# briangodwinlim/SIR-GCN

Measured on AMD Instinct MI355X. Metric: edges/sec SIRConv fwd+bwd, d_hidden=256, 1/2/4/8 MI355X, higher is better.
Workload: dtype f32; 1 GPU; cfg4 S2: Chung-Lu power-law V=2000000 E=40000000 alpha=0.8; 1 SIRConv layer d_in=H=d_out=256, agg=sum, LeakyReLU(0.2), f32, feat_dropout=0.0; fwd+bwd incl. projections; graph=S2, V=2000000, E=40000000, hidden=256, agg=sum, parallelism=single GPU

## Files before the change

### sir-gcn_amd/csrc/sirconv_gemm.hip

```cpp
#include <type_traits>
#include <algorithm>

#include "sirconv_internal.h"
#include "sirconv_gemm_util.h"
#include "sirconv_dropout.h"

namespace sir {
namespace {
using namespace gemm;

typedef _Float16 h8 __attribute__((ext_vector_type(8)));
typedef float f16v __attribute__((ext_vector_type(16)));
typedef unsigned int u4v __attribute__((ext_vector_type(4)));

constexpr int KC = 32;

#ifndef SIR_HR
#define SIR_HR 8
#endif

__device__ inline int bexp(float m) { return (int)((__float_as_uint(m) >> 23) & 255u) - 126; }
__device__ inline int scale_exp(int e) { int s = 15 - e; return s > 126 ? 126 : s; }
constexpr int SE_INIT = 127;
__device__ inline int next_se(int se_old, int e_c) {
    if (e_c + se_old <= 15) return se_old;
    const int s = 15 - SIR_HR - e_c;
    return s > 126 ? 126 : s;
}
__device__ inline void kahan_add(float& s, float& c, float x) {
    const float y = x - c;
    const float t = s + y;
    c = (t - s) - y;
    s = t;
}
__device__ inline float pow2(int e) { e = e < -126 ? -126 : (e > 127 ? 127 : e); return __uint_as_float((uint32_t)(e + 127) << 23); }
__device__ inline void drop4(const Drop& d, int64_t row, int n, float4& o) {
    const uint32_t rh = drop_row_hash(d, row);
    const int c = d.col0 + n;
    o.x = drop_keep(d, rh, c + 0) ? o.x * d.scale : 0.f;
    o.y = drop_keep(d, rh, c + 1) ? o.y * d.scale : 0.f;
    o.z = drop_keep(d, rh, c + 2) ? o.z * d.scale : 0.f;
    o.w = drop_keep(d, rh, c + 3) ? o.w * d.scale : 0.f;
}

__device__ inline float gate_dact(float g, float x, int relu, float slope) {
    return g > 0.f ? x : (relu ? 0.f : x * slope);
}
__global__ void __launch_bounds__(256)
k_gate_dact_bits(float* __restrict__ C, int64_t ldc, const uint64_t* __restrict__ mask, int64_t M, int relu, float slope) {
    const int64_t i = (int64_t)blockIdx.x * 256 + threadIdx.x;
    if (i >= M * 256) return;
    const int64_t r = i >> 8;
    const int c = (int)(i & 255);
    const bool pos = (mask[r * 4 + (c & 3)] >> (c >> 2)) & 1u;
    C[r * ldc + c] = gate_dact(pos ? 1.f : -1.f, C[r * ldc + c], relu, slope);
}
__global__ void __launch_bounds__(256)
k_gate_dact(float* __restrict__ C, int64_t ldc, const float* __restrict__ gate, int64_t M, int N, int relu, float slope) {
    const int64_t i = (int64_t)blockIdx.x * 256 + threadIdx.x;
    if (i >= M * N) return;
    const int64_t r = i / N, c = i % N;
    C[r * ldc + c] = gate_dact(gate[r * ldc + c], C[r * ldc + c], relu, slope);
}

__device__ inline void split8_mix(float4 a, float4 b, float s, h8& hi, h8& lo) {
    uint32_t h0, h1, h2, h3, l0, l1, l2, l3;
    asm volatile(
        "v_fma_mixlo_f16 %0, %8, %16, 0\n\tv_fma_mixhi_f16 %0, %9, %16, 0\n\t"
        "v_fma_mixlo_f16 %1, %10, %16, 0\n\tv_fma_mixhi_f16 %1, %11, %16, 0\n\t"
        "v_fma_mixlo_f16 %2, %12, %16, 0\n\tv_fma_mixhi_f16 %2, %13, %16, 0\n\t"
        "v_fma_mixlo_f16 %3, %14, %16, 0\n\tv_fma_mixhi_f16 %3, %15, %16, 0\n\t"
        "v_fma_mixlo_f16 %4, %8, %16, -%0 op_sel_hi:[0,0,1]\n\tv_fma_mixhi_f16 %4, %9, %16, -%0 op_sel:[0,0,1] op_sel_hi:[0,0,1]\n\t"
        "v_fma_mixlo_f16 %5, %10, %16, -%1 op_sel_hi:[0,0,1]\n\tv_fma_mixhi_f16 %5, %11, %16, -%1 op_sel:[0,0,1] op_sel_hi:[0,0,1]\n\t"
        "v_fma_mixlo_f16 %6, %12, %16, -%2 op_sel_hi:[0,0,1]\n\tv_fma_mixhi_f16 %6, %13, %16, -%2 op_sel:[0,0,1] op_sel_hi:[0,0,1]\n\t"
        "v_fma_mixlo_f16 %7, %14, %16, -%3 op_sel_hi:[0,0,1]\n\tv_fma_mixhi_f16 %7, %15, %16, -%3 op_sel:[0,0,1] op_sel_hi:[0,0,1]\n\t"
        "s_nop 1"
        : "=&v"(h0), "=&v"(h1), "=&v"(h2), "=&v"(h3), "=&v"(l0), "=&v"(l1), "=&v"(l2), "=&v"(l3)
        : "v"(a.x), "v"(a.y), "v"(a.z), "v"(a.w), "v"(b.x), "v"(b.y), "v"(b.z), "v"(b.w), "v"(s));
    typedef uint32_t u4 __attribute__((ext_vector_type(4)));
    hi = __builtin_bit_cast(h8, u4{h0, h1, h2, h3});
    lo = __builtin_bit_cast(h8, u4{l0, l1, l2, l3});
}
#define SIR_SPLIT1(x, i) { const float y_ = (x) * s; const _Float16 h_ = (_Float16)y_; hi[i] = h_; lo[i] = (_Float16)(y_ - (float)h_); }
__device__ inline void split8(float4 a, float4 b, float s, h8& hi, h8& lo) {
    SIR_SPLIT1(a.x, 0) SIR_SPLIT1(a.y, 1) SIR_SPLIT1(a.z, 2) SIR_SPLIT1(a.w, 3)
    SIR_SPLIT1(b.x, 4) SIR_SPLIT1(b.y, 5) SIR_SPLIT1(b.z, 6) SIR_SPLIT1(b.w, 7)
}
#undef SIR_SPLIT1

__device__ inline float fmax4_mix(float m, float4 v) {
    asm("v_max3_f32 %0, %0, |%1|, |%2|\n\tv_max3_f32 %0, %0, |%3|, |%4|" : "+v"(m) : "v"(v.x), "v"(v.y), "v"(v.z), "v"(v.w));
    return m;
}
__device__ inline float fmax4(float m, float4 v) {
    return fmaxf(fmaxf(m, fmaxf(fabsf(v.x), fabsf(v.y))), fmaxf(fabsf(v.z), fabsf(v.w)));
}

__global__ void __launch_bounds__(64)
k_pack_weight(const float* __restrict__ W, int64_t ldw, int N, int K, int trans, int Npad, int Kc,
              _Float16* __restrict__ out, float* __restrict__ inv_scale) {
    const int n = blockIdx.x, l = threadIdx.x;
    float m = 0.f;
    if (n < N)
        for (int k = l; k < K; k += 64) m = fmaxf(m, fabsf(trans ? W[(int64_t)k * ldw + n] : W[(int64_t)n * ldw + k]));
#pragma unroll
    for (int o = 32; o > 0; o >>= 1) m = fmaxf(m, __shfl_xor(m, o));
    const int se = scale_exp(bexp(m));
    const float s = pow2(se);
    for (int k = l; k < Kc * KC; k += 64) {
        float x = 0.f;
        if (n < N && k < K) x = trans ? W[(int64_t)k * ldw + n] : W[(int64_t)n * ldw + k];
        const float y = x * s;
        const _Float16 h = (_Float16)y;
        const int kc = k / KC, ks = (k / 16) & 1, j = k & 15;
        const int64_t at = fimg(n, j >> 3) / 2 + (j & 7);
        out[(((int64_t)kc * 2 + 0) * 2 + ks) * Npad * 16 + at] = h;
        out[(((int64_t)kc * 2 + 1) * 2 + ks) * Npad * 16 + at] = (_Float16)(y - (float)h);
    }
    if (l == 0) inv_scale[n] = (n < N) ? pow2(-se) : 0.f;
}

template <int WD, int WF, int TDT, int TFT, bool KFULL>
__global__ void __launch_bounds__(64 * WD * WF)
k_gemm_nt(const float* __restrict__ A, int64_t lda, int64_t M, int K,
          const u4v* __restrict__ Wp, int Npad, const float* __restrict__ inv_t,
          const float* __restrict__ bias, int N, float* __restrict__ C, int64_t ldc, int n_ftiles, Drop drop) {
    drop = drop_resolve(drop);
    constexpr int NT = 64 * WD * WF;
    constexpr int BD = 32 * TDT * WD;
    constexpr int BF = 32 * TFT * WF;
    constexpr int TPR = NT / BD;
    static_assert(TPR == 1 || TPR == 2 || TPR == 4, "loader mapping");
    constexpr int FPT = KC / TPR;
    constexpr int WPT = BF * 8 / NT;
    static_assert(WPT >= 1 && BF * 8 % NT == 0, "weight loader mapping");
    constexpr int D_BYTES = BD * 128, W_BYTES = BF * 128;
    constexpr int STAGE = D_BYTES + W_BYTES + BD * 4;
    __shared__ __attribute__((aligned(16))) char lds[2 * STAGE];

    const int t = threadIdx.x;
    const int wg = xcd_remap(blockIdx.x, gridDim.x);
    const int64_t d0 = (int64_t)(wg / n_ftiles) * BD;
    const int f0 = (wg % n_ftiles) * BF;
    const int nc = (K + KC - 1) / KC;

    const int rho = t / TPR, kp = t % TPR;
    const int64_t rows_here = (M - d0 < BD) ? M - d0 : BD;
    const rsrc_t arsrc = mk_rsrc(A + d0 * lda, (uint32_t)(rows_here * lda * 4));
    const int aoff = (rho * (int)lda + kp * FPT) * 4;
    const rsrc_t wrsrc = mk_rsrc(Wp, (uint32_t)((int64_t)nc * Npad * 128));
    int woff[WPT];
#pragma unroll
    for (int i = 0; i < WPT; ++i) {
        const int p = t + i * NT;
        const int plane = p / (BF * 2), rem = p % (BF * 2);
        const int nl = (rem >> 6) * 32 + (rem & 31), q = (rem >> 5) & 1;
        woff[i] = plane * Npad * 32 + fimg(f0 + nl, q);
    }
    int se_run = SE_INIT;

    const int w = t >> 6, l = t & 63, r = l & 31, h = l >> 5;
    const int d_w = (w / WF) * TDT * 32, f_w = (w % WF) * TFT * 32;

    float4 dv[2][FPT / 4];
    u4v wv[WPT];

    auto load_a = [&](int set, int c) {
#pragma unroll
        for (int i = 0; i < FPT / 4; ++i) {
            const int k = c * KC + kp * FPT + 4 * i;
            const u4v u = __builtin_amdgcn_raw_buffer_load_b128(arsrc, aoff + 16 * i, c * KC * 4, 0);
            dv[set][i] = (KFULL || k < K) ? make_float4(__uint_as_float(u.x), __uint_as_float(u.y), __uint_as_float(u.z),
                                               __uint_as_float(u.w))
                                 : make_float4(0.f, 0.f, 0.f, 0.f);
        }
    };
// ... 89 lines not shown
    store(0, 0, true);
    auto step_full = [&](int c, int set) {
        compute(c & 1);
        store(set, (c & 1) ^ 1);
        load_w(c + 2);
        load_a(set, c + 3);
        __syncthreads();
    };
    auto step_tail = [&](int c, int set) {
        compute(c & 1);
        if (c + 1 < nc) {
            store(set, (c & 1) ^ 1);
            if (c + 2 < nc) load_w(c + 2);
            if (c + 3 < nc) load_a(set, c + 3);
        }
        __syncthreads();
    };
    int c = 0;
    if (nc > 4) {
        load_a(1, 1);
        load_w(1);
        load_a(0, 2);
        __syncthreads();
        for (; c + 4 < nc; c += 2) {
            step_full(c, 1);
            step_full(c + 1, 0);
        }
    } else {
        if (nc > 1) { load_a(1, 1); load_w(1); }
        if (nc > 2) load_a(0, 2);
        __syncthreads();
    }
    for (; c < nc; c += 2) {
        step_tail(c, 1);
        if (c + 1 < nc) step_tail(c + 1, 0);
    }

    constexpr int RR = WD * 32, PITCH = BF * 4 + 16;
    constexpr int SC_OFF = STAGE + D_BYTES + W_BYTES;
    static_assert(RR * PITCH <= SC_OFF, "epilogue image overlaps the scale row");
    static_assert((RR * BF / 4) % NT == 0, "epilogue copy mapping");
    float* sc = reinterpret_cast<float*>(lds + SC_OFF);
    if (kp == 0) sc[rho] = pow2(-se_run);
    __syncthreads();
#pragma unroll
    for (int b = 0; b < TDT; ++b) {
        const int dl = d_w + 32 * b + r;
        const float is = sc[dl];
        char* rowp = lds + ((w / WF) * 32 + r) * PITCH;
#pragma unroll
        for (int a = 0; a < TFT; ++a) {
#pragma unroll
            for (int g = 0; g < 4; ++g) {
                const int nl = f_w + 32 * a + 8 * g + 4 * h;
                const int n = f0 + nl;
                const float4 it = *reinterpret_cast<const float4*>(inv_t + n);
                float4 o;
                o.x = acc[a][b][4 * g + 0] * is * it.x;
                o.y = acc[a][b][4 * g + 1] * is * it.y;
                o.z = acc[a][b][4 * g + 2] * is * it.z;
                o.w = acc[a][b][4 * g + 3] * is * it.w;
                if (bias != nullptr && n < N) {
                    const float4 bb = *reinterpret_cast<const float4*>(bias + n);
                    o.x += bb.x; o.y += bb.y; o.z += bb.z; o.w += bb.w;
                }
                if (drop.on()) drop4(drop, d0 + dl, n, o);
                *reinterpret_cast<float4*>(rowp + nl * 4) = o;
            }
        }
        __syncthreads();
#pragma unroll
        for (int k = 0; k < RR * BF / 4 / NT; ++k) {
            const int idx = t + k * NT;
            const int row = idx / (BF / 4), c4 = idx % (BF / 4);
            const int64_t m = d0 + (row >> 5) * (TDT * 32) + 32 * b + (row & 31);
            const int n = f0 + c4 * 4;
            const float4 o = *reinterpret_cast<const float4*>(lds + row * PITCH + c4 * 16);
            if (m < M && n < N) *reinterpret_cast<float4*>(C + m * ldc + n) = o;
        }
        __syncthreads();
    }
}

constexpr int NT_P_NMAX = 512;

template <int NCT, int GATE>
__global__ void __launch_bounds__(512)
k_gemm_nt_p(const float* __restrict__ A, int64_t lda, int64_t M, const u4v* __restrict__ Wp, int Npad,
            const float* __restrict__ inv_t, const float* __restrict__ bias, int N, float* __restrict__ C,
            int64_t ldc, int n_ftiles, int n_tiles, int tiles_per_block, Drop drop, const float* __restrict__ gate,
            int gate_relu, float gate_slope) {
    drop = drop_resolve(drop);
    constexpr int WF = 4, TDT = 4, TFT = 2;
    constexpr int NT = 512, BD = 256, BF = 256, TPR = NT / BD, FPT = KC / TPR, WPT = BF * 8 / NT;
    static_assert(TPR == 2 && WPT == 4 && NCT >= 4 && NCT % 2 == 0, "mapping");
    constexpr int D_BYTES = BD * 128, W_BYTES = BF * 128;
    constexpr int STAGE = D_BYTES + W_BYTES + BD * 4;
    constexpr int FIN_OFF = 2 * STAGE;
    constexpr int EPI_OFF = FIN_OFF + 2 * BD * 4;
    __shared__ __attribute__((aligned(16))) char lds[EPI_OFF + 2 * NT_P_NMAX * 4];

    const int t = threadIdx.x;
    const int tb = blockIdx.x * tiles_per_block;
    const int te = (tb + tiles_per_block < n_tiles) ? tb + tiles_per_block : n_tiles;
    if (tb >= te) return;
    float* const inv_l = reinterpret_cast<float*>(lds + EPI_OFF);
    float* const bias_l = inv_l + NT_P_NMAX;
    float* const fin = reinterpret_cast<float*>(lds + FIN_OFF);
    for (int n = t; n < Npad; n += NT) {
        inv_l[n] = inv_t[n];
        bias_l[n] = (bias != nullptr && n < N) ? bias[n] : -0.f;
    }

    const int rho = t / TPR, kp = t % TPR;
    const int aoff = (rho * (int)lda + kp * FPT) * 4;
    const rsrc_t wrsrc = mk_rsrc(Wp, (uint32_t)((int64_t)NCT * Npad * 128));
    static_assert(BF * 2 == NT, "one weight plane per loader pass");
    const int woff = fimg((t >> 6) * 32 + (t & 31), (t >> 5) & 1);
    struct TileP { rsrc_t a; int64_t d0; int f0; int rows; };
    auto tile_p = [&](int tt) {
        TileP p;
        if (tt < te) {
            p.d0 = (int64_t)(tt / n_ftiles) * BD;
            p.f0 = (tt % n_ftiles) * BF;
            p.rows = (M - p.d0 < BD) ? (int)(M - p.d0) : BD;
            p.a = mk_rsrc(A + p.d0 * lda, (uint32_t)(p.rows * lda * 4));
        } else {
            p.d0 = 0;
            p.f0 = 0;
            p.rows = 0;
            p.a = mk_rsrc(A, 0u);
        }
        return p;
    };
    int se_run = SE_INIT;

    const int w = t >> 6, l = t & 63, r = l & 31, h = l >> 5;
    const int d_w = (w / WF) * TDT * 32, f_w = (w % WF) * TFT * 32;

    float4 dv[2][FPT / 4];
    u4v wv[WPT];
    auto load_a = [&](int set, const TileP& p, int c) {
#pragma unroll
        for (int i = 0; i < FPT / 4; ++i) {
            const u4v u = __builtin_amdgcn_raw_buffer_load_b128(p.a, aoff + 16 * i, c * KC * 4, 0);
            dv[set][i] = make_float4(__uint_as_float(u.x), __uint_as_float(u.y), __uint_as_float(u.z),
                                     __uint_as_float(u.w));
        }
    };
    auto load_w = [&](const TileP& p, int c) {
#pragma unroll
        for (int i = 0; i < WPT; ++i)
            wv[i] = __builtin_amdgcn_raw_buffer_load_b128(wrsrc, woff, c * Npad * 128 + i * Npad * 32 + p.f0 * 32, 0);
    };
    auto store = [&](int set, int buf, bool first, bool last, int slot) {
        char* st = lds + buf * STAGE;
        float m = 0.f;
#pragma unroll
        for (int i = 0; i < FPT / 4; ++i) m = fmax4_mix(m, dv[set][i]);
        m = fmaxf(m, __shfl_xor(m, 1));
        const int se_old = first ? SE_INIT : se_run, se = next_se(se_old, bexp(m));
        se_run = se;
        const float s = pow2(se);
#pragma unroll
        for (int j = 0; j < FPT; j += 8) {
            const int kl = kp * FPT + j, ks = kl >> 4, pos = kl & 15;
            h8 hv, lv;
// ... 890 lines not shown
            if (do_cs) tile.step<true>(x0, x1, h);
            else tile.step<false>(x0, x1, h);
        }
        SIR_LT_TRACE_AT(5 + 2 * (s & 7), __builtin_amdgcn_s_memtime());
    }
    SIR_LT_TRACE_AT(3, __builtin_amdgcn_s_memtime());
    float pv[16];
    tile.result(pv, h);
    wait_vm<0>();
    __syncthreads();
    float* red = lds;
    float* cred = lds + G::RED;
    const int tile_id = w0 + W0 * w1;
    if (wk > 0) {
#pragma unroll
        for (int i = 0; i < 16; ++i) red[(((wk - 1) * W0 * W1 + tile_id) * 16 + i) * 64 + l] = pv[i];
    }
    if (do_cs) cred[(wk * G::L0 + w0 * 32 + j) * 2 + h] = tile.cs;
    __syncthreads();
    if (wk == 0) {
#pragma unroll
        for (int q = 1; q < WK; ++q) {
#pragma unroll
            for (int i = 0; i < 16; ++i) pv[i] += red[(((q - 1) * W0 * W1 + tile_id) * 16 + i) * 64 + l];
        }
        const int64_t r1 = a1 + 32 * w1 + j;
        if constexpr (EPI == 0) {
            if (r1 < n1lines) {
#pragma unroll
                for (int g = 0; g < 4; ++g) {
                    const int64_t n = a0 + 32 * w0 + 8 * g + 4 * h;
                    if (n < n0lines) {
                        float4 o = make_float4(pv[4 * g] + bb[g].x, pv[4 * g + 1] + bb[g].y, pv[4 * g + 2] + bb[g].z,
                                               pv[4 * g + 3] + bb[g].w);
                        if (drop.on()) drop4(drop, r1, (int)n, o);
                        *reinterpret_cast<float4*>(C + r1 * ldc + n) = o;
                    }
                }
            }
        } else {
            float* out = C + p * n0lines * n1lines;
            if (r1 < n1lines) {
#pragma unroll
                for (int i = 0; i < 16; ++i) {
                    const int64_t m = a0 + 32 * w0 + (i & 3) + 8 * (i >> 2) + 4 * h;
                    if (m < n0lines) out[m * n1lines + r1] = pv[i];
                }
            }
        }
    }
    SIR_LT_TRACE_AT(20, __builtin_amdgcn_s_memtime());
    SIR_LT_TRACE_AT(21, __builtin_amdgcn_s_memrealtime());
    if (do_cs && t < G::L0 && a0 + t < n0lines) {
        float sum = 0.f;
#pragma unroll
        for (int q = 0; q < WK; ++q) sum += cred[(q * G::L0 + t) * 2] + cred[(q * G::L0 + t) * 2 + 1];
        csum_part[p * n0lines + a0 + t] = sum;
    }
}

}

#ifndef SIR_SMALL_ROWS
#define SIR_SMALL_ROWS 16384
#endif
static int64_t gemm_small_rows() {
    const char* e = getenv("SIR_GEMM_SMALL_ROWS");
    return (e != nullptr && e[0] != 0) ? atoll(e) : (int64_t)SIR_SMALL_ROWS;
}

#ifndef SIR_TN_S_ROWS
#define SIR_TN_S_ROWS 512
#endif
#ifndef SIR_LT_NT
#define SIR_LT_NT -1
#endif
#ifndef SIR_LT_TN
#define SIR_LT_TN 2
#endif
static int lt_env(const char* name, int dflt) {
    const char* e = getenv(name);
    return (e != nullptr && e[0] != 0) ? atoi(e) : dflt;
}
#ifndef SIR_LT_BLOCKS
#define SIR_LT_BLOCKS 512
#endif
static bool aligned16(const void* p, int64_t ld) { return ((uintptr_t)p & 15u) == 0 && ld % 4 == 0; }
static int gemm_tn_splits_lt(int64_t R, int64_t tiles, int KS, int64_t* rps) {
    int64_t P = (SIR_LT_BLOCKS + tiles - 1) / tiles;
    const int64_t pmax = (R + KS - 1) / KS;
    if (P > pmax) P = pmax;
    if (P > 32) P = 32;
    if (P < 1) P = 1;
    int64_t r = (R + P - 1) / P;
    r = (r + KS - 1) / KS * KS;
    *rps = r > 0 ? r : KS;
    P = (R + *rps - 1) / *rps;
    return (int)(P < 1 ? 1 : P);
}

static int gemm_tn_splits_s(int64_t R, int64_t, int64_t) {
    int64_t P = (R + SIR_TN_S_ROWS - 1) / SIR_TN_S_ROWS;
    if (P > 16) P = 16;
    if (P < 1) P = 1;
    return (int)P;
}

static hipError_t run_gemm_nt_s(const float* A, int64_t lda, int64_t M, int K, const void* packed, int N,
                                const float* bias, float* C, int64_t ldc, hipStream_t st, const Drop& drop) {
    const int np = (int)gemm_pack_npad(N), kc = (K + KC - 1) / KC;
    const u4v* wp = static_cast<const u4v*>(packed);
    const float* inv = reinterpret_cast<const float*>(static_cast<const char*>(packed) + (int64_t)kc * 4 * np * 32);
    const int nfg = (N + 32 * S_FT - 1) / (32 * S_FT);
    const int64_t waves = (M + 31) / 32 * nfg;
    const unsigned blocks = (unsigned)((waves + 3) / 4);
    if (K % KC == 0)
        hipLaunchKernelGGL(k_gemm_nt_s<true>, dim3(blocks), dim3(256), 0, st, A, lda, M, K, wp, np, kc, inv, bias, N, C,
                           ldc, nfg, waves, drop);
    else
        hipLaunchKernelGGL(k_gemm_nt_s<false>, dim3(blocks), dim3(256), 0, st, A, lda, M, K, wp, np, kc, inv, bias, N, C,
                           ldc, nfg, waves, drop);
    return hipGetLastError();
}

#ifndef SIR_LT_NS
#define SIR_LT_NS 3
#endif
struct NtW {
    const float* W;
    int64_t ldw;
    const float* W2;
    int64_t ldw2, split, bias_cols;
};
template <bool TRANS, int W0, int W1, int WK>
static void launch_nt_lt(const float* A, int64_t lda, int64_t M, int K, const NtW& w, int N, const float* bias,
                         float* C, int64_t ldc, hipStream_t st, const Drop& drop) {
    using G = Lt<!TRANS, true, W0, W1, WK, SIR_LT_NS>;
    const int nt0 = (N + G::L0 - 1) / G::L0;
    const int64_t nt1 = (M + G::L1 - 1) / G::L1;
    hipLaunchKernelGGL((k_gemm_lt<!TRANS, true, W0, W1, WK, SIR_LT_NS, 0>), dim3((unsigned)(nt0 * nt1)), dim3(G::NT), 0, st,
                       w.W, w.ldw, A, lda, (int64_t)N, M, (int64_t)K, nt0, (int)nt1, (int64_t)K, bias, C, ldc, nullptr,
                       drop, w.W2, w.ldw2, w.split, w.bias_cols);
}

static int nt_lt_auto(int64_t M, int N) {
    const int64_t ncu = device_cu_count();
    if ((int64_t)((N + 31) / 32) * ((M + 63) / 64) <= ncu) return 7;
    if ((int64_t)((N + 63) / 64) * ((M + 63) / 64) <= ncu) return 8;
    return 3;
}

hipError_t run_gemm_nt_direct(const float* A, int64_t lda, int64_t M, int K, const float* W, int64_t ldw, int trans,
                              int N, const float* bias, float* C, int64_t ldc, hipStream_t st, const Drop& drop,
                              const float* W2, int64_t ldw2, int64_t split, int64_t bias_cols) {
    if (M == 0 || N == 0) return hipSuccess;
    int lt = lt_env("SIR_LT_NT", SIR_LT_NT);
    if (lt < 0) lt = nt_lt_auto(M, N);
    const NtW w{W, ldw, W2, ldw2, W2 != nullptr ? split : INT64_MAX, bias_cols};
    if (lt > 0 && K % 4 == 0 && N % 4 == 0 && aligned16(A, lda) && aligned16(W, ldw) && ((uintptr_t)bias & 15u) == 0
        && (W2 == nullptr || aligned16(W2, ldw2)) && 128 * lda < ((int64_t)1 << 29)
        && (trans ? (int64_t)K * ldw : 128 * ldw) < ((int64_t)1 << 29)
        && (M + 31) / 32 * ((N + 31) / 32) < ((int64_t)1 << 31)) {
        switch (lt * 2 + (trans ? 1 : 0)) {
        case 2: launch_nt_lt<false, 2, 2, 1>(A, lda, M, K, w, N, bias, C, ldc, st, drop); break;
        case 3: launch_nt_lt<true, 2, 2, 1>(A, lda, M, K, w, N, bias, C, ldc, st, drop); break;
        case 4: launch_nt_lt<false, 1, 2, 2>(A, lda, M, K, w, N, bias, C, ldc, st, drop); break;
// ... 11 lines not shown
        case 16: launch_nt_lt<false, 2, 2, 2>(A, lda, M, K, w, N, bias, C, ldc, st, drop); break;
        case 17: launch_nt_lt<true, 2, 2, 2>(A, lda, M, K, w, N, bias, C, ldc, st, drop); break;
        default: return hipErrorInvalidValue;
        }
        return hipGetLastError();
    }
    if (W2 != nullptr || bias_cols < N) return hipErrorInvalidValue;
    const int nft = (N + 31) / 32;
    const int64_t blocks = (M + 31) / 32 * nft;
    if (trans)
        hipLaunchKernelGGL(k_gemm_nt_sw<true>, dim3((unsigned)blocks), dim3(256), 0, st, A, lda, M, K, W, ldw, N, bias, C,
                           ldc, nft, drop);
    else
        hipLaunchKernelGGL(k_gemm_nt_sw<false>, dim3((unsigned)blocks), dim3(256), 0, st, A, lda, M, K, W, ldw, N, bias,
                           C, ldc, nft, drop);
    return hipGetLastError();
}

int64_t gemm_pack_npad(int64_t N) { return (N + 255) / 256 * 256; }
int64_t gemm_pack_bytes(int64_t N, int64_t K) {
    const int64_t np = gemm_pack_npad(N), kc = (K + KC - 1) / KC;
    return (kc * 4 * np * 32 + np * 4 + 15) / 16 * 16;
}

hipError_t run_gemm_pack(const float* W, int64_t ldw, int N, int K, int trans, void* packed, hipStream_t st) {
    const int np = (int)gemm_pack_npad(N), kc = (K + KC - 1) / KC;
    _Float16* out = static_cast<_Float16*>(packed);
    float* inv = reinterpret_cast<float*>(static_cast<char*>(packed) + (int64_t)kc * 4 * np * 32);
    hipLaunchKernelGGL(k_pack_weight, dim3(np), dim3(64), 0, st, W, ldw, N, K, trans, np, kc, out, inv);
    return hipGetLastError();
}

template <int GATE>
static bool launch_gemm_nt_p(const float* A, int64_t lda, int64_t M, int kc, const void* packed, int N,
                             const float* bias, float* C, int64_t ldc, hipStream_t st, const Drop& drop,
                             const float* gate, int gate_relu, float gate_slope) {
    const int np = (int)gemm_pack_npad(N);
    const u4v* wp = static_cast<const u4v*>(packed);
    const float* inv = reinterpret_cast<const float*>(static_cast<const char*>(packed) + (int64_t)kc * 4 * np * 32);
    constexpr int BD = 256, BF = 256;
    const int nft = (N + BF - 1) / BF;
    const int64_t ntiles = (M + BD - 1) / BD * nft;
    const int ncu = device_cu_count();
    if (ntiles >= (int64_t)1 << 30) return false;
    const int tpb = (int)((ntiles + ncu - 1) / ncu);
    const int nblk = (int)((ntiles + tpb - 1) / tpb);
    auto kern = kc == 4 ? k_gemm_nt_p<4, GATE> : (kc == 8 ? k_gemm_nt_p<8, GATE> : k_gemm_nt_p<16, GATE>);
    hipLaunchKernelGGL(kern, dim3((unsigned)nblk), dim3(512), 0, st, A, lda, M, wp, np, inv, bias, N, C, ldc, nft,
                       (int)ntiles, tpb, drop, gate, gate_relu, gate_slope);
    return true;
}

hipError_t run_gemm_nt(const float* A, int64_t lda, int64_t M, int K, const void* packed, int N,
                       const float* bias, float* C, int64_t ldc, hipStream_t st, const Drop& drop, const float* gate,
                       int gate_relu, float gate_slope, const uint64_t* gate_mask) {
    if (M == 0 || N == 0) return hipSuccess;
    if (gate_mask != nullptr && N != 256) return hipErrorInvalidValue;
    if (gate != nullptr || gate_mask != nullptr) {
        const int np = (int)gemm_pack_npad(N), kc = (K + KC - 1) / KC;
        if (M >= gemm_small_rows() && N > 128 && np <= NT_P_NMAX && K % KC == 0 && (kc == 4 || kc == 8 || kc == 16)) {
            const bool done =
                gate_mask != nullptr
                    ? launch_gemm_nt_p<2>(A, lda, M, kc, packed, N, bias, C, ldc, st, drop,
                                          reinterpret_cast<const float*>(gate_mask), gate_relu, gate_slope)
                    : launch_gemm_nt_p<1>(A, lda, M, kc, packed, N, bias, C, ldc, st, drop, gate, gate_relu, gate_slope);
            if (done) return hipGetLastError();
        }
        hipError_t err = run_gemm_nt(A, lda, M, K, packed, N, bias, C, ldc, st, drop, nullptr, 0, 0.f, nullptr);
        if (err != hipSuccess) return err;
        const int64_t cnt = M * N;
        if (gate_mask != nullptr)
            hipLaunchKernelGGL(k_gate_dact_bits, dim3((unsigned)((cnt + 255) / 256)), dim3(256), 0, st, C, ldc, gate_mask, M,
                               gate_relu, gate_slope);
        else
            hipLaunchKernelGGL(k_gate_dact, dim3((unsigned)((cnt + 255) / 256)), dim3(256), 0, st, C, ldc, gate, M, N,
                               gate_relu, gate_slope);
        return hipGetLastError();
    }
    const int np = (int)gemm_pack_npad(N), kc = (K + KC - 1) / KC;
    const u4v* wp = static_cast<const u4v*>(packed);
    const float* inv = reinterpret_cast<const float*>(static_cast<const char*>(packed) + (int64_t)kc * 4 * np * 32);
    const bool kfull = K % KC == 0;
    if (M < gemm_small_rows()) return run_gemm_nt_s(A, lda, M, K, packed, N, bias, C, ldc, st, drop);
    if (N > 128 && np <= NT_P_NMAX && kfull && (kc == 4 || kc == 8 || kc == 16) &&
        launch_gemm_nt_p<0>(A, lda, M, kc, packed, N, bias, C, ldc, st, drop, nullptr, 0, 0.f))
        return hipGetLastError();
    if (N > 128) {
        constexpr int BD = 256, BF = 256;
        const int nft = (N + BF - 1) / BF;
        const int64_t nblk = (M + BD - 1) / BD * nft;
        if (kfull)
            hipLaunchKernelGGL((k_gemm_nt<2, 4, 4, 2, true>), dim3((unsigned)nblk), dim3(512), 0, st,
                               A, lda, M, K, wp, np, inv, bias, N, C, ldc, nft, drop);
        else
            hipLaunchKernelGGL((k_gemm_nt<2, 4, 4, 2, false>), dim3((unsigned)nblk), dim3(512), 0, st,
                               A, lda, M, K, wp, np, inv, bias, N, C, ldc, nft, drop);
    } else {
        constexpr int BD = 256, BF = 128;
        const int nft = (N + BF - 1) / BF;
        const int64_t nblk = (M + BD - 1) / BD * nft;
        if (kfull)
            hipLaunchKernelGGL((k_gemm_nt<4, 2, 2, 2, true>), dim3((unsigned)nblk), dim3(512), 0, st,
                               A, lda, M, K, wp, np, inv, bias, N, C, ldc, nft, drop);
        else
            hipLaunchKernelGGL((k_gemm_nt<4, 2, 2, 2, false>), dim3((unsigned)nblk), dim3(512), 0, st,
                               A, lda, M, K, wp, np, inv, bias, N, C, ldc, nft, drop);
    }
    return hipGetLastError();
}

hipError_t run_gemm_reduce(const float* part, int P, int64_t count, int Nc, float* C, int64_t ldc, hipStream_t st) {
    if (count > 0)
        hipLaunchKernelGGL(k_gemm_reduce, dim3((unsigned)((count + 255) / 256)), dim3(256), 0, st, part, P, count, Nc, C,
                           ldc);
    return hipGetLastError();
}

#ifndef SIR_TN_MINROWS
#define SIR_TN_MINROWS 1024
#endif
int gemm_tn_splits(int64_t R, int64_t Mc, int64_t Nc) {
    const int64_t tiles = ((Mc + 255) / 256) * ((Nc + 255) / 256);
    int64_t P = (256 + tiles - 1) / tiles;
    const int64_t pmax = (R + SIR_TN_MINROWS - 1) / SIR_TN_MINROWS;
    if (P > pmax) P = pmax;
    if (P < 1) P = 1;
    return (int)P;
}

int64_t gemm_tn_workspace(int64_t R, int64_t Mc, int64_t Nc) {
    int64_t P = gemm_tn_splits(R, Mc, Nc);
    if (R < gemm_small_rows()) {
        const int64_t ps = gemm_tn_splits_s(R, Mc, Nc);
        if (ps > P) P = ps;
        if (P < 32) P = 32;
    }
    return P * (Mc * Nc + Mc) * 4;
}

static int lt_tn_w0(int lt) { return (lt == 1 || lt == 5) ? 2 : 1; }
static int lt_tn_w1(int lt) { return lt == 3 ? 1 : 2; }
static int lt_tn_ks(int lt) { return 32 * (lt == 1 ? 1 : (lt == 2 || lt == 5) ? 2 : 4); }
static int64_t lt_tn_tiles(int lt, int Mc, int Nc) {
    const int a = 32 * lt_tn_w0(lt), b = 32 * lt_tn_w1(lt);
    return (int64_t)((Mc + a - 1) / a) * ((Nc + b - 1) / b);
}
template <int W0, int W1, int WK>
static void launch_tn_lt(const float* A, int64_t lda, const float* B, int64_t ldb, int64_t R, int Mc, int Nc,
                         float* part, bool colsum, hipStream_t st) {
    using G = Lt<false, false, W0, W1, WK, SIR_LT_NS>;
    const int nt0 = (Mc + G::L0 - 1) / G::L0, nt1 = (Nc + G::L1 - 1) / G::L1;
    const int64_t tiles = (int64_t)nt0 * nt1;
    int64_t rl = 0;
    const int Pl = gemm_tn_splits_lt(R, tiles, G::KS, &rl);
    float* cp = colsum ? part + (int64_t)Pl * Mc * Nc : nullptr;
    hipLaunchKernelGGL((k_gemm_lt<false, false, W0, W1, WK, SIR_LT_NS, 1>), dim3((unsigned)(Pl * tiles)), dim3(G::NT), 0,
                       st, A, lda, B, ldb, (int64_t)Mc, (int64_t)Nc, R, nt0, nt1, rl, nullptr, part, (int64_t)0, cp,
                       Drop{});
}

hipError_t run_gemm_tn(const float* A, int64_t lda, const float* B, int64_t ldb, int64_t R, int Mc, int Nc,
                       float* C, int64_t ldc, float* colsum, void* workspace, hipStream_t st) {
    if (Mc == 0 || Nc == 0) return hipSuccess;
    const bool small = R < gemm_small_rows();
    const int P = small ? gemm_tn_splits_s(R, Mc, Nc) : gemm_tn_splits(R, Mc, Nc);
    const int64_t rps = (R + P - 1) / P;
    const int nmt = (Mc + 255) / 256, nnt = (Nc + 255) / 256;
// ... 37 lines not shown
```

Measured before the change: 1.918 billion edges/s.

## Add two-blocks-per-CU persistent NT GEMM variant with smaller row tiles

Adds a new persistent NT GEMM kernel with 256 threads, 128-row tiles and launch bounds allowing two blocks per CU. Weights are streamed straight from global memory into registers instead of being staged in LDS, and the epilogue goes through an LDS image with buffer stores. Shared helpers move into a header. The kernel is picked automatically for K/N shapes of 256/512, aiming for better latency hiding through higher occupancy, at the cost of more register pressure and weight reloads per block.

```diff
diff --git a/sir-gcn_amd/csrc/sirconv_gemm.hip b/sir-gcn_amd/csrc/sirconv_gemm.hip
--- a/sir-gcn_amd/csrc/sirconv_gemm.hip
+++ b/sir-gcn_amd/csrc/sirconv_gemm.hip
@@ -4,43 +4,17 @@
 #include "sirconv_internal.h"
 #include "sirconv_gemm_util.h"
 #include "sirconv_dropout.h"
+#include "sirconv_gemm_nt.h"
 
 namespace sir {
 namespace {
 using namespace gemm;
 
-typedef _Float16 h8 __attribute__((ext_vector_type(8)));
-typedef float f16v __attribute__((ext_vector_type(16)));
-typedef unsigned int u4v __attribute__((ext_vector_type(4)));
-
-constexpr int KC = 32;
-
-#ifndef SIR_HR
-#define SIR_HR 8
-#endif
-
-__device__ inline int bexp(float m) { return (int)((__float_as_uint(m) >> 23) & 255u) - 126; }
-__device__ inline int scale_exp(int e) { int s = 15 - e; return s > 126 ? 126 : s; }
-constexpr int SE_INIT = 127;
-__device__ inline int next_se(int se_old, int e_c) {
-    if (e_c + se_old <= 15) return se_old;
-    const int s = 15 - SIR_HR - e_c;
-    return s > 126 ? 126 : s;
-}
 __device__ inline void kahan_add(float& s, float& c, float x) {
     const float y = x - c;
     const float t = s + y;
     c = (t - s) - y;
     s = t;
-}
-__device__ inline float pow2(int e) { e = e < -126 ? -126 : (e > 127 ? 127 : e); return __uint_as_float((uint32_t)(e + 127) << 23); }
-__device__ inline void drop4(const Drop& d, int64_t row, int n, float4& o) {
-    const uint32_t rh = drop_row_hash(d, row);
-    const int c = d.col0 + n;
-    o.x = drop_keep(d, rh, c + 0) ? o.x * d.scale : 0.f;
-    o.y = drop_keep(d, rh, c + 1) ? o.y * d.scale : 0.f;
-    o.z = drop_keep(d, rh, c + 2) ? o.z * d.scale : 0.f;
-    o.w = drop_keep(d, rh, c + 3) ? o.w * d.scale : 0.f;
 }
 
 __device__ inline float gate_dact(float g, float x, int relu, float slope) {
@@ -63,24 +37,6 @@
     C[r * ldc + c] = gate_dact(gate[r * ldc + c], C[r * ldc + c], relu, slope);
 }
 
-__device__ inline void split8_mix(float4 a, float4 b, float s, h8& hi, h8& lo) {
-    uint32_t h0, h1, h2, h3, l0, l1, l2, l3;
-    asm volatile(
-        "v_fma_mixlo_f16 %0, %8, %16, 0\n\tv_fma_mixhi_f16 %0, %9, %16, 0\n\t"
-        "v_fma_mixlo_f16 %1, %10, %16, 0\n\tv_fma_mixhi_f16 %1, %11, %16, 0\n\t"
-        "v_fma_mixlo_f16 %2, %12, %16, 0\n\tv_fma_mixhi_f16 %2, %13, %16, 0\n\t"
-        "v_fma_mixlo_f16 %3, %14, %16, 0\n\tv_fma_mixhi_f16 %3, %15, %16, 0\n\t"
-        "v_fma_mixlo_f16 %4, %8, %16, -%0 op_sel_hi:[0,0,1]\n\tv_fma_mixhi_f16 %4, %9, %16, -%0 op_sel:[0,0,1] op_sel_hi:[0,0,1]\n\t"
-        "v_fma_mixlo_f16 %5, %10, %16, -%1 op_sel_hi:[0,0,1]\n\tv_fma_mixhi_f16 %5, %11, %16, -%1 op_sel:[0,0,1] op_sel_hi:[0,0,1]\n\t"
-        "v_fma_mixlo_f16 %6, %12, %16, -%2 op_sel_hi:[0,0,1]\n\tv_fma_mixhi_f16 %6, %13, %16, -%2 op_sel:[0,0,1] op_sel_hi:[0,0,1]\n\t"
-        "v_fma_mixlo_f16 %7, %14, %16, -%3 op_sel_hi:[0,0,1]\n\tv_fma_mixhi_f16 %7, %15, %16, -%3 op_sel:[0,0,1] op_sel_hi:[0,0,1]\n\t"
-        "s_nop 1"
-        : "=&v"(h0), "=&v"(h1), "=&v"(h2), "=&v"(h3), "=&v"(l0), "=&v"(l1), "=&v"(l2), "=&v"(l3)
-        : "v"(a.x), "v"(a.y), "v"(a.z), "v"(a.w), "v"(b.x), "v"(b.y), "v"(b.z), "v"(b.w), "v"(s));
-    typedef uint32_t u4 __attribute__((ext_vector_type(4)));
-    hi = __builtin_bit_cast(h8, u4{h0, h1, h2, h3});
-    lo = __builtin_bit_cast(h8, u4{l0, l1, l2, l3});
-}
 #define SIR_SPLIT1(x, i) { const float y_ = (x) * s; const _Float16 h_ = (_Float16)y_; hi[i] = h_; lo[i] = (_Float16)(y_ - (float)h_); }
 __device__ inline void split8(float4 a, float4 b, float s, h8& hi, h8& lo) {
     SIR_SPLIT1(a.x, 0) SIR_SPLIT1(a.y, 1) SIR_SPLIT1(a.z, 2) SIR_SPLIT1(a.w, 3)
@@ -88,10 +44,6 @@
 }
 #undef SIR_SPLIT1
 
-__device__ inline float fmax4_mix(float m, float4 v) {
-    asm("v_max3_f32 %0, %0, |%1|, |%2|\n\tv_max3_f32 %0, %0, |%3|, |%4|" : "+v"(m) : "v"(v.x), "v"(v.y), "v"(v.z), "v"(v.w));
-    return m;
-}
 __device__ inline float fmax4(float m, float4 v) {
     return fmaxf(fmaxf(m, fmaxf(fabsf(v.x), fabsf(v.y))), fmaxf(fabsf(v.z), fabsf(v.w)));
 }
@@ -347,7 +299,6 @@
     }
 }
 
-constexpr int NT_P_NMAX = 512;
 
 template <int NCT, int GATE>
 __global__ void __launch_bounds__(512)
@@ -1404,6 +1355,12 @@
     const char* e = getenv(name);
     return (e != nullptr && e[0] != 0) ? atoi(e) : dflt;
 }
+#ifndef SIR_NT_2B
+#define SIR_NT_2B -1
+#endif
+static bool nt_2b_auto(int K, int N) {
+    return (K == 256 && (N == 256 || N == 512)) || (K == 512 && N == 256);
+}
 #ifndef SIR_LT_BLOCKS
 #define SIR_LT_BLOCKS 512
 #endif
@@ -1581,7 +1538,12 @@
     const float* inv = reinterpret_cast<const float*>(static_cast<const char*>(packed) + (int64_t)kc * 4 * np * 32);
     const bool kfull = K % KC == 0;
     if (M < gemm_small_rows()) return run_gemm_nt_s(A, lda, M, K, packed, N, bias, C, ldc, st, drop);
-    if (N > 128 && np <= NT_P_NMAX && kfull && (kc == 4 || kc == 8 || kc == 16) &&
+    const bool persistent = N > 128 && np <= NT_P_NMAX && kfull && (kc == 4 || kc == 8 || kc == 16);
+    const int two = lt_env("SIR_NT_2B", SIR_NT_2B);
+    if (persistent && (two < 0 ? nt_2b_auto(K, N) : two != 0) &&
+        launch_gemm_nt_p2(A, lda, M, kc, packed, N, bias, C, ldc, st, drop))
+        return hipGetLastError();
+    if (persistent &&
         launch_gemm_nt_p<0>(A, lda, M, kc, packed, N, bias, C, ldc, st, drop, nullptr, 0, 0.f))
         return hipGetLastError();
     if (N > 128) {
diff --git a/sir-gcn_amd/csrc/sirconv_gemm_nt.h b/sir-gcn_amd/csrc/sirconv_gemm_nt.h
--- /dev/null
+++ b/sir-gcn_amd/csrc/sirconv_gemm_nt.h
@@ -0,0 +1,69 @@
+#pragma once
+#include "sirconv_internal.h"
+#include "sirconv_gemm_util.h"
+#include "sirconv_dropout.h"
+
+namespace sir {
+namespace gemm {
+
+typedef _Float16 h8 __attribute__((ext_vector_type(8)));
+typedef float f16v __attribute__((ext_vector_type(16)));
+typedef unsigned int u4v __attribute__((ext_vector_type(4)));
+
+constexpr int KC = 32;
+
+#ifndef SIR_HR
+#define SIR_HR 8
+#endif
+
+__device__ inline int bexp(float m) { return (int)((__float_as_uint(m) >> 23) & 255u) - 126; }
+__device__ inline int scale_exp(int e) { int s = 15 - e; return s > 126 ? 126 : s; }
+constexpr int SE_INIT = 127;
+__device__ inline int next_se(int se_old, int e_c) {
+    if (e_c + se_old <= 15) return se_old;
+    const int s = 15 - SIR_HR - e_c;
+    return s > 126 ? 126 : s;
+}
+__device__ inline float pow2(int e) { e = e < -126 ? -126 : (e > 127 ? 127 : e); return __uint_as_float((uint32_t)(e + 127) << 23); }
+__device__ inline void drop4(const Drop& d, int64_t row, int n, float4& o) {
+    const uint32_t rh = drop_row_hash(d, row);
+    const int c = d.col0 + n;
+    o.x = drop_keep(d, rh, c + 0) ? o.x * d.scale : 0.f;
+    o.y = drop_keep(d, rh, c + 1) ? o.y * d.scale : 0.f;
+    o.z = drop_keep(d, rh, c + 2) ? o.z * d.scale : 0.f;
+    o.w = drop_keep(d, rh, c + 3) ? o.w * d.scale : 0.f;
+}
+
+__device__ inline void split8_mix(float4 a, float4 b, float s, h8& hi, h8& lo) {
+    uint32_t h0, h1, h2, h3, l0, l1, l2, l3;
+    asm volatile(
+        "v_fma_mixlo_f16 %0, %8, %16, 0\n\tv_fma_mixhi_f16 %0, %9, %16, 0\n\t"
+        "v_fma_mixlo_f16 %1, %10, %16, 0\n\tv_fma_mixhi_f16 %1, %11, %16, 0\n\t"
+        "v_fma_mixlo_f16 %2, %12, %16, 0\n\tv_fma_mixhi_f16 %2, %13, %16, 0\n\t"
+        "v_fma_mixlo_f16 %3, %14, %16, 0\n\tv_fma_mixhi_f16 %3, %15, %16, 0\n\t"
+        "v_fma_mixlo_f16 %4, %8, %16, -%0 op_sel_hi:[0,0,1]\n\tv_fma_mixhi_f16 %4, %9, %16, -%0 op_sel:[0,0,1] op_sel_hi:[0,0,1]\n\t"
+        "v_fma_mixlo_f16 %5, %10, %16, -%1 op_sel_hi:[0,0,1]\n\tv_fma_mixhi_f16 %5, %11, %16, -%1 op_sel:[0,0,1] op_sel_hi:[0,0,1]\n\t"
+        "v_fma_mixlo_f16 %6, %12, %16, -%2 op_sel_hi:[0,0,1]\n\tv_fma_mixhi_f16 %6, %13, %16, -%2 op_sel:[0,0,1] op_sel_hi:[0,0,1]\n\t"
+        "v_fma_mixlo_f16 %7, %14, %16, -%3 op_sel_hi:[0,0,1]\n\tv_fma_mixhi_f16 %7, %15, %16, -%3 op_sel:[0,0,1] op_sel_hi:[0,0,1]\n\t"
+        "s_nop 1"
+        : "=&v"(h0), "=&v"(h1), "=&v"(h2), "=&v"(h3), "=&v"(l0), "=&v"(l1), "=&v"(l2), "=&v"(l3)
+        : "v"(a.x), "v"(a.y), "v"(a.z), "v"(a.w), "v"(b.x), "v"(b.y), "v"(b.z), "v"(b.w), "v"(s));
+    typedef uint32_t u4 __attribute__((ext_vector_type(4)));
+    hi = __builtin_bit_cast(h8, u4{h0, h1, h2, h3});
+    lo = __builtin_bit_cast(h8, u4{l0, l1, l2, l3});
+}
+
+__device__ inline float fmax4_mix(float m, float4 v) {
+    asm("v_max3_f32 %0, %0, |%1|, |%2|\n\tv_max3_f32 %0, %0, |%3|, |%4|" : "+v"(m) : "v"(v.x), "v"(v.y), "v"(v.z), "v"(v.w));
+    return m;
+}
+
+constexpr int NT_P_NMAX = 512;
+
+}
+
+int64_t gemm_pack_npad(int64_t N);
+bool launch_gemm_nt_p2(const float* A, int64_t lda, int64_t M, int kc, const void* packed, int N, const float* bias,
+                       float* C, int64_t ldc, hipStream_t st, const Drop& drop);
+
+}
diff --git a/sir-gcn_amd/csrc/sirconv_gemm_nt2.hip b/sir-gcn_amd/csrc/sirconv_gemm_nt2.hip
--- /dev/null
+++ b/sir-gcn_amd/csrc/sirconv_gemm_nt2.hip
@@ -0,0 +1,276 @@
+#include <type_traits>
+
+#include "sirconv_gemm_nt.h"
+
+namespace sir {
+namespace {
+using namespace gemm;
+
+__device__ __forceinline__ void lds_barrier() { asm volatile("s_waitcnt lgkmcnt(0)\n\ts_barrier" ::: "memory"); }
+
+template <int NCT>
+__global__ void __launch_bounds__(256, 2)
+k_gemm_nt_p2(const float* __restrict__ A, int64_t lda, int64_t M, const u4v* __restrict__ Wp, int Npad,
+             const float* __restrict__ inv_t, const float* __restrict__ bias, int N, float* __restrict__ C,
+             int64_t ldc, int n_ftiles, int n_tiles, int tiles_per_block, Drop drop) {
+    drop = drop_resolve(drop);
+    constexpr int TDT = 4, TFT = 2;
+    constexpr int NT = 256, BD = 128, BF = 256, TPR = NT / BD, FPT = KC / TPR;
+    static_assert(TPR == 2 && NCT >= 4 && NCT % 2 == 0, "mapping");
+    constexpr int D_BYTES = BD * 128;
+    constexpr int ASTAGE = D_BYTES + BD * 4;
+    constexpr int FIN_OFF = 2 * ASTAGE;
+    constexpr int EPI_OFF = FIN_OFF + 2 * BD * 4;
+    constexpr int IMG_OFF = EPI_OFF + 2 * NT_P_NMAX * 4;
+    constexpr int PITCH = BF * 4 + 16;
+    constexpr int LDS_BYTES = IMG_OFF + 32 * PITCH;
+    static_assert(2 * LDS_BYTES <= 160 * 1024 && LDS_BYTES <= 78 * 1024, "two blocks per CU");
+    __shared__ __attribute__((aligned(16))) char lds[LDS_BYTES];
+
+    const int t = threadIdx.x;
+    const int bid = xcd_remap((int)blockIdx.x, (int)gridDim.x);
+    const int tb = bid * tiles_per_block;
+    const int te = (tb + tiles_per_block < n_tiles) ? tb + tiles_per_block : n_tiles;
+    if (tb >= te) return;
+    float* const inv_l = reinterpret_cast<float*>(lds + EPI_OFF);
+    float* const bias_l = inv_l + NT_P_NMAX;
+    float* const fin = reinterpret_cast<float*>(lds + FIN_OFF);
+    for (int n = t; n < Npad; n += NT) {
+        inv_l[n] = inv_t[n];
+        bias_l[n] = (bias != nullptr && n < N) ? bias[n] : -0.f;
+    }
+
+    const int rho = t / TPR, kp = t % TPR;
+    const int aoff = (rho * (int)lda + kp * FPT) * 4;
+    struct TileP { rsrc_t a; int64_t d0; int f0; int rows; };
+    auto tile_p = [&](int tt) {
+        TileP p;
+        if (tt < te) {
+            p.d0 = (int64_t)(tt / n_ftiles) * BD;
+            p.f0 = (tt % n_ftiles) * BF;
+            p.rows = (M - p.d0 < BD) ? (int)(M - p.d0) : BD;
+            p.a = mk_rsrc(A + p.d0 * lda, (uint32_t)(p.rows * lda * 4));
+        } else {
+            p.d0 = 0;
+            p.f0 = 0;
+            p.rows = 0;
+            p.a = mk_rsrc(A, 0u);
+        }
+        return p;
+    };
+    int se_run = SE_INIT;
+
+    const int w = t >> 6, l = t & 63, r = l & 31, h = l >> 5;
+    const int f_w = w * TFT * 32;
+    const int wvoff = f_w * 32 + l * 16;
+    const rsrc_t wrsrc = mk_rsrc(Wp, (uint32_t)((int64_t)NCT * Npad * 128));
+
+    float4 dv[2][FPT / 4];
+    auto load_a = [&](int set, const TileP& p, int c) {
+#pragma unroll
+        for (int i = 0; i < FPT / 4; ++i) {
+            const u4v u = __builtin_amdgcn_raw_buffer_load_b128(p.a, aoff + 16 * i, c * KC * 4, 0);
+            dv[set][i] = make_float4(__uint_as_float(u.x), __uint_as_float(u.y), __uint_as_float(u.z),
+                                     __uint_as_float(u.w));
+        }
+    };
+    u4v wv[2][TFT][2];
+    auto load_w = [&](const TileP& p, int c, int ks) {
+#pragma unroll
+        for (int pt = 0; pt < 2; ++pt)
+#pragma unroll
+            for (int a = 0; a < TFT; ++a)
+                wv[ks][a][pt] = __builtin_amdgcn_raw_buffer_load_b128(
+                    wrsrc, wvoff, (((c * 2 + pt) * 2 + ks) * Npad + p.f0 + 32 * a) * 32, 0);
+    };
+    auto store = [&](int set, int buf, bool first, bool last, int slot) {
+        char* st = lds + buf * ASTAGE;
+        float m = 0.f;
+#pragma unroll
+        for (int i = 0; i < FPT / 4; ++i) m = fmax4_mix(m, dv[set][i]);
+        m = fmaxf(m, __shfl_xor(m, 1));
+        const int se_old = first ? SE_INIT : se_run, se = next_se(se_old, bexp(m));
+        se_run = se;
+        const float s = pow2(se);
+#pragma unroll
+        for (int j = 0; j < FPT; j += 8) {
+            const int kl = kp * FPT + j, ks = kl >> 4, pos = kl & 15;
+            h8 hv, lv;
+            split8_mix(dv[set][j / 4], dv[set][j / 4 + 1], s, hv, lv);
+            *reinterpret_cast<h8*>(st + (0 * 2 + ks) * BD * 32 + fimg(rho, pos >> 3)) = hv;
+            *reinterpret_cast<h8*>(st + (1 * 2 + ks) * BD * 32 + fimg(rho, pos >> 3)) = lv;
+        }
+        reinterpret_cast<float*>(st + D_BYTES)[rho] = first ? 1.f : pow2(se - se_old);
+        if (last) {
+            int rq = threadIdx.x;
+            asm volatile("" : "+v"(rq));
+            fin[slot * BD + rq / TPR] = pow2(-se);
+        }
+    };
+
+    f16v acc[TFT][TDT];
+    auto rescale = [&](int buf) {
+        const float* fac = reinterpret_cast<const float*>(lds + buf * ASTAGE + D_BYTES);
+        float f[TDT];
+        bool ch = false;
+#pragma unroll
+        for (int b = 0; b < TDT; ++b) { f[b] = fac[32 * b + r]; ch |= f[b] != 1.f; }
+        if (__builtin_amdgcn_ballot_w64(ch) != 0) {
+#pragma unroll
+            for (int b = 0; b < TDT; ++b)
+#pragma unroll
+                for (int a = 0; a < TFT; ++a) acc[a][b] *= f[b];
+        }
+    };
+    auto mfma_ks = [&](int buf, int ks, bool zinit) {
+        const char* st = lds + buf * ASTAGE;
+        const f16v zero = {};
+        h8 wf[TFT][2], df[TDT][2];
+#pragma unroll
+        for (int pt = 0; pt < 2; ++pt) {
+#pragma unroll
+            for (int a = 0; a < TFT; ++a) wf[a][pt] = __builtin_bit_cast(h8, wv[ks][a][pt]);
+#pragma unroll
+            for (int b = 0; b < TDT; ++b)
+                df[b][pt] = *reinterpret_cast<const h8*>(st + (pt * 2 + ks) * BD * 32 + fimg(32 * b + r, h));
+        }
+#pragma unroll
+        for (int a = 0; a < TFT; ++a)
+#pragma unroll
+            for (int b = 0; b < TDT; ++b)
+                acc[a][b] = __builtin_amdgcn_mfma_f32_32x32x16_f16(wf[a][0], df[b][0], zinit ? zero : acc[a][b], 0, 0, 0);
+#pragma unroll
+        for (int a = 0; a < TFT; ++a)
+#pragma unroll
+            for (int b = 0; b < TDT; ++b)
+                acc[a][b] = __builtin_amdgcn_mfma_f32_32x32x16_f16(wf[a][0], df[b][1], acc[a][b], 0, 0, 0);
+#pragma unroll
+        for (int a = 0; a < TFT; ++a)
+#pragma unroll
+            for (int b = 0; b < TDT; ++b)
+                acc[a][b] = __builtin_amdgcn_mfma_f32_32x32x16_f16(wf[a][1], df[b][0], acc[a][b], 0, 0, 0);
+    };
+    constexpr int EPI_VM = TDT * 8;
+    auto epilogue = [&](const TileP& p, int slot) {
+        int tq = threadIdx.x;
+        asm volatile("" : "+v"(tq));
+        const int lq = tq & 63, rq = lq & 31, hq = lq >> 5, wq = tq >> 6;
+        const int f_wq = wq * TFT * 32;
+        char* const img = lds + IMG_OFF;
+        const uint32_t ldc4 = (uint32_t)ldc * 4u;
+        const uint32_t nrec = (uint32_t)p.rows * ldc4;
+        const rsrc_t crs = mk_rsrc(C + p.d0 * ldc, nrec);
+        const float* sc = fin + slot * BD;
+        char* const wrow = img + rq * PITCH + (f_wq + 4 * hq) * 4;
+#pragma unroll
+        for (int b = 0; b < TDT; ++b) {
+            const float is = sc[32 * b + rq];
+#pragma unroll
+            for (int a = 0; a < TFT; ++a) {
+#pragma unroll
+                for (int g = 0; g < 4; ++g) {
+                    const int n = p.f0 + f_wq + 32 * a + 8 * g + 4 * hq;
+                    const float4 it = *reinterpret_cast<const float4*>(inv_l + n);
+                    const float4 bb = *reinterpret_cast<const float4*>(bias_l + n);
+                    float4 o;
+                    o.x = acc[a][b][4 * g + 0] * is * it.x + bb.x;
+                    o.y = acc[a][b][4 * g + 1] * is * it.y + bb.y;
+                    o.z = acc[a][b][4 * g + 2] * is * it.z + bb.z;
+                    o.w = acc[a][b][4 * g + 3] * is * it.w + bb.w;
+                    if (drop.on()) drop4(drop, p.d0 + 32 * b + rq, n, o);
+                    *reinterpret_cast<float4*>(wrow + (32 * a + 8 * g) * 4) = o;
+                }
+            }
+            lds_barrier();
+#pragma unroll
+            for (int i = 0; i < 8; ++i) {
+                const int ir = wq + 4 * i, c16 = lq;
+                const u4v v = *reinterpret_cast<const u4v*>(img + ir * PITCH + c16 * 16);
+                const int ml = 32 * b + ir;
+                const uint32_t off = (p.f0 + 4 * c16 < N) ? (uint32_t)ml * ldc4 + (uint32_t)c16 * 16u : nrec;
+                __builtin_amdgcn_raw_buffer_store_b128(v, crs, off, p.f0 * 4, 0);
+                __builtin_amdgcn_sched_barrier(0);
+                asm volatile("s_nop 1" ::: "memory");
+                __builtin_amdgcn_sched_barrier(0);
+            }
+            if (b + 1 < TDT) lds_barrier();
+        }
+    };
+
+    TileP cur = tile_p(tb), nxt = tile_p(tb + 1);
+    load_a(0, cur, 0);
+    store(0, 0, true, false, 0);
+    load_a(1, cur, 1);
+    load_w(cur, 0, 0);
+    load_w(cur, 0, 1);
+    load_a(0, cur, 2);
+    {
+        const rsrc_t nul = mk_rsrc(C, 0u);
+#pragma unroll
+        for (int i = 0; i < EPI_VM; ++i) {
+            __builtin_amdgcn_raw_buffer_store_b128(u4v{0u, 0u, 0u, 0u}, nul, 16 * i, 0, 0);
+        }
+    }
+    lds_barrier();
+    typedef std::integral_constant<int, 0> I0;
+    typedef std::integral_constant<int, 1> I1;
+    typedef std::integral_constant<int, 2> I2;
+    auto step = [&](int c, int j, const TileP& cu, const TileP& nx, auto P_, auto Z_, auto SK_, auto WN_, auto AN_) {
+        constexpr int P = decltype(P_)::value, SK = decltype(SK_)::value;
+        constexpr bool Z = decltype(Z_)::value != 0, WN = decltype(WN_)::value != 0, AN = decltype(AN_)::value != 0;
+        if constexpr (!Z) rescale(P);
+        mfma_ks(P, 0, Z);
+        if constexpr (SK == 2) store(0, 0, true, false, 0);
+        else store(P ^ 1, P ^ 1, false, SK == 1, j & 1);
+        if constexpr (WN) load_w(nx, c + 1 - NCT, 0);
+        else load_w(cu, c + 1, 0);
+        __builtin_amdgcn_sched_barrier(0);
+        mfma_ks(P, 1, false);
+        if constexpr (WN) load_w(nx, c + 1 - NCT, 1);
+        else load_w(cu, c + 1, 1);
+        if constexpr (AN) load_a(P ^ 1, nx, c + 3 - NCT);
+        else load_a(P ^ 1, cu, c + 3);
+        lds_barrier();
+    };
+    auto run = [&]() {
+        TileP cu = cur, nx = nxt;
+        for (int j = 0; tb + j < te; ++j) {
+            const TileP nn = tile_p(tb + j + 2);
+            step(0, j, cu, nx, I0(), I1(), I0(), I0(), I0());
+#pragma unroll
+            for (int c = 1; c + 1 <= NCT - 4; c += 2) {
+                step(c, j, cu, nx, I1(), I0(), I0(), I0(), I0());
+                step(c + 1, j, cu, nx, I0(), I0(), I0(), I0(), I0());
+            }
+            step(NCT - 3, j, cu, nx, I1(), I0(), I0(), I0(), I1());
+            step(NCT - 2, j, cu, nx, I0(), I0(), I1(), I0(), I1());
+            step(NCT - 1, j, cu, nx, I1(), I0(), I2(), I1(), I1());
+            epilogue(cu, j & 1);
+            cu = nx;
+            nx = nn;
+        }
+    };
+    run();
+}
+
+}
+
+bool launch_gemm_nt_p2(const float* A, int64_t lda, int64_t M, int kc, const void* packed, int N, const float* bias,
+                       float* C, int64_t ldc, hipStream_t st, const Drop& drop) {
+    const int np = (int)gemm_pack_npad(N);
+    const u4v* wp = static_cast<const u4v*>(packed);
+    const float* inv = reinterpret_cast<const float*>(static_cast<const char*>(packed) + (int64_t)kc * 4 * np * 32);
+    constexpr int BD = 128, BF = 256;
+    const int nft = (N + BF - 1) / BF;
+    const int64_t ntiles = (M + BD - 1) / BD * nft;
+    if (ntiles >= (int64_t)1 << 30) return false;
+    const int nmax = 2 * device_cu_count();
+    const int tpb = (int)((ntiles + nmax - 1) / nmax);
+    const int nblk = (int)((ntiles + tpb - 1) / tpb);
+    auto kern = kc == 4 ? k_gemm_nt_p2<4> : (kc == 8 ? k_gemm_nt_p2<8> : k_gemm_nt_p2<16>);
+    hipLaunchKernelGGL(kern, dim3((unsigned)nblk), dim3(256), 0, st, A, lda, M, wp, np, inv, bias, N, C, ldc, nft,
+                       (int)ntiles, tpb, drop);
+    return true;
+}
+
+}
```

Result: faster. 1.939 billion edges/s, median of 6 (+1.1%).
